# cmavro/GNN-RAG

Hardware: AMD Instinct MI355X
Metric: kg_edges_aggregated_per_sec (higher is better)
Workload: dtype f32

## Files before the change

### gnn-rag_amd/csrc/dense_internal.h

```cpp
#pragma once
#include "gnnrag_common.h"

namespace gnnrag {

int tables_vq_launch_z(const gnnrag_csr* csr, const void* planes, const float* ins, const float* W, float* P, int32_t D,
                       int32_t I, int32_t only_dir, float* zero, int64_t zero_n, hipStream_t stream);

int tables_vq_lite_launch_z(const gnnrag_csr* csr, const void* planes, const float* ins, const float* W, float* P, int32_t D,
                            int32_t I, int32_t only_dir, float* zero, int64_t zero_n, hipStream_t stream);

int update_b3_launch_z(const float* h, const float* nbr, const float* W, const float* b, const float* w_s,
                       const float* b_s, const float* mask, float* h_out, float* score, int64_t BN, int32_t D,
                       int32_t ldw, hipStream_t stream, bool score_zeroed);

int update_score_fused_rows(const float* h, const float* nbr, const uint8_t* add_flag, const float* W, const float* b,
                            const float* w_s, const float* b_s, const float* mask, float* h_out, float* score,
                            int64_t BN, int32_t D, int32_t I, int32_t math, hipStream_t stream, bool score_zeroed);
int update_b3_launch_f(const float* h, const float* nbr, const uint8_t* add_flag, const float* W, const float* b,
                       const float* w_s, const float* b_s, const float* mask, float* h_out, float* score, int64_t BN,
                       int32_t D, int32_t ldw, hipStream_t stream, bool score_zeroed);

bool update_rows_supported(const float* h, const float* nbr, const float* W, const float* h_out, int64_t BN, int32_t D,
                           int32_t I, int32_t math);
bool update_b3_shape_ok(int64_t BN, int32_t D, int32_t ldw);
int tables_small_launch(const gnnrag_csr* csr, const float* T_fwd, const float* T_inv, const float* ins, const float* W,
                        float* P, int32_t D, int32_t I, hipStream_t stream);

int frontier_build_z(const gnnrag_csr* csr, const float* dist, void* fws, size_t fws_bytes, float* zero_a,
                     int64_t zero_na, float* zero_b, int64_t zero_nb, hipStream_t stream);
const uint8_t* frontier_row_flags(const gnnrag_csr* csr, const void* fws);

int update_score_fused_z(const float* h, const float* nbr, const float* W, const float* b, const float* w_s,
                         const float* b_s, const float* mask, float* h_out, float* score, int64_t BN, int32_t D,
                         int32_t I, int32_t math, hipStream_t stream, bool score_zeroed);

bool rel_transform_accepts(const float* relfeat_fwd, const float* relfeat_inv, int64_t R1, int32_t D, int32_t L,
                           const gnnrag_layer_params* layers, int32_t pos_rows, const float* T_out, const void* planes_out);

}
```

### gnn-rag_amd/csrc/gemm_f32.hip

```cpp
#include "gnnrag_common.h"
#include "dense_internal.h"

#define GNNRAG_GEMM_MT1_NW 8
#ifndef GNNRAG_UPDATE_B3
#define GNNRAG_UPDATE_B3 1
#endif
#ifndef GNNRAG_TABLES_WRES
#define GNNRAG_TABLES_WRES 1
#endif
#ifndef GNNRAG_GEMM_WRES
#define GNNRAG_GEMM_WRES 1
#endif
#ifndef GNNRAG_UPDATE_SKINNY
#define GNNRAG_UPDATE_SKINNY 1
#endif

namespace gnnrag {


constexpr int kBK = 32;
constexpr int kSkinnyMaxM = 16384;

enum { EPI_LINEAR = 0, EPI_UPDATE = 1 };

// ... 705 lines not shown
  for (int nt = 0; nt < NT; ++nt) wrow[nt] = g.W + (size_t)min(nt * 16 + fr, Nout - 1) * g.ldw + g.wc0;
  for (int k0 = 0; k0 < K; k0 += 32) {
    f32x4 a[2], b[2][NT];
#pragma unroll
    for (int c = 0; c < 2; ++c) {
      const int k = k0 + c * 16 + fg * 4;
      const bool ok = k < K;
      a[c] = ok ? *reinterpret_cast<const f32x4*>(arow + k) : zero4;
#pragma unroll
      for (int nt = 0; nt < NT; ++nt) b[c][nt] = ok ? *reinterpret_cast<const f32x4*>(wrow[nt] + k) : zero4;
    }
#pragma unroll
    for (int c = 0; c < 2; ++c)
#pragma unroll
      for (int nt = 0; nt < NT; ++nt)
#pragma unroll
        for (int e = 0; e < 4; ++e) acc[nt] = __builtin_amdgcn_mfma_f32_16x16x4f32(a[c][e], b[c][nt][e], acc[nt], 0, 0, 0);
  }
  const int rbase = m0 + 4 * fg;
  unsigned fl = 0x01010101u;
  if (g.add_flag) fl = *reinterpret_cast<const unsigned*>(g.add_flag + rbase);
  float part[4] = {0.f, 0.f, 0.f, 0.f};
#pragma unroll
  for (int nt = 0; nt < NT; ++nt) {
    const int col = nt * 16 + fr;
    const bool cok = col < Nout;
    const float bia = (cok && g.bias) ? g.bias[col] : 0.f;
    const float wsc = cok ? g.w_s[col] : 0.f;
#pragma unroll
    for (int q = 0; q < 4; ++q) {
      const int row = rbase + q;
      float v = 0.f;
      if (cok && row < g.M) {
        float ad = 0.f;
        if (g.add && ((fl >> (8 * q)) & 0xffu)) ad = g.add[(size_t)row * Nout + col];
        v = fmaxf((acc[nt][q] + bia) + ad, 0.f);
        g.C[(size_t)row * Nout + col] = v;
      }
      part[q] += v * wsc;
    }
  }
  const float tot = row16_sum4(part, lane);
  const int srow = rbase + row16_sum4_index(fr);
  if (fr < 4 && srow < g.M) g.score[srow] = (tot + g.b_s[0]) + (1.0f - g.mask[srow]) * kVeryNeg;
}

static bool update_skinny_ok(const GemmArgs& g) {
  return g.M < 4096 && !g.A1 && g.K == g.K0 && g.K % 4 == 0 && g.Nout <= 208 && g.ldw % 4 == 0 && g.wc0 % 4 == 0 &&
         aligned16(g.A0) && aligned16(g.W) && (!g.add || g.add_rows >= g.M) &&
         (!g.add_flag || ((uintptr_t)g.add_flag & 3) == 0);
}

static int launch_update_skinny(const GemmArgs& g, hipStream_t stream) {
  const int nt = (g.Nout + 15) / 16;
  const dim3 grid((unsigned)(((g.M + 15) / 16 + 3) / 4));
#define GNNRAG_USK(N) case N: hipLaunchKernelGGL((k_update_skinny<N>), grid, dim3(256), 0, stream, g); break;
  switch (nt) {
    GNNRAG_USK(1) GNNRAG_USK(2) GNNRAG_USK(3) GNNRAG_USK(4) GNNRAG_USK(5) GNNRAG_USK(6) GNNRAG_USK(7) GNNRAG_USK(8)
    GNNRAG_USK(9) GNNRAG_USK(10) GNNRAG_USK(11) GNNRAG_USK(12) GNNRAG_USK(13)
    default: return GNNRAG_E_UNSUPPORTED;
  }
#undef GNNRAG_USK
  GNNRAG_LAUNCH_CHECK();
  return 0;
}

static bool math_ok(int math) { return math == GNNRAG_MATH_FP32 || math == GNNRAG_MATH_BF16X3 || math == GNNRAG_MATH_MIXED; }

template <int EPI, int AMODE>
static int launch_gemm(GemmArgs g, hipStream_t stream, int math) {
  if (g.M <= 0) return 0;
  const bool v4 = (g.K % 4 == 0) && (g.K0 % 4 == 0) && (g.ldw % 4 == 0) && (g.wc0 % 4 == 0) &&
                  aligned16(g.A0) && aligned16(g.W) && (g.A1 == nullptr || aligned16(g.A1)) &&
                  (g.C_b == nullptr || aligned16(g.A0b)) &&
                  (AMODE != AMODE_GEN || g.gen_D % 4 == 0);
  if (EPI == EPI_LINEAR && AMODE == AMODE_PLAIN && g.M <= kSkinnyMaxM && g.n0 == 0) {
    const dim3 grid((g.M + 15) / 16, (g.Nout + 255) / 256, g.C_b ? 2 : 1);
    if (v4) hipLaunchKernelGGL((k_gemm_skinny<true>), grid, dim3(256), 0, stream, g);
    else hipLaunchKernelGGL((k_gemm_skinny<false>), grid, dim3(256), 0, stream, g);
    GNNRAG_LAUNCH_CHECK();
    return 1 << 30;
  }
  const int ny = AMODE == AMODE_GEN ? 2 : 1;
  const int tiles128 = ((g.M + 127) / 128) * ny;
  const bool small_tiles = tiles128 < 1024;
  const int slots8 = 512;
  const int t8 = tiles128;
  const bool nw8 = small_tiles && (t8 >= 3 * slots8 / 2 || (t8 % slots8 == 0) || (t8 % slots8) > slots8 / 2) &&
                   GNNRAG_GEMM_MT1_NW == 8;
  const int bm = small_tiles ? (nw8 ? 128 : 64) : 128;
  const dim3 grid((g.M + bm - 1) / bm, ny);
  const int ncol = g.Nout - g.n0;
  const bool b3 = math != GNNRAG_MATH_FP32;
  g.v4out = (g.Nout % 4 == 0) && (g.n0 % 4 == 0) && aligned16(g.C) && (g.add == nullptr || aligned16(g.add));
#define GNNRAG_GEMM_LAUNCH(NT, MT, V, MATH, NW) \
  hipLaunchKernelGGL((k_gemm_f32<NT, MT, V, EPI, AMODE, MATH, NW>), grid, dim3(64 * NW), 0, stream, g)
#define GNNRAG_GEMM_CASE(NT)                                                        \
  do {                                                                              \
    if (small_tiles && nw8) {                                                       \
      if (v4 && b3) GNNRAG_GEMM_LAUNCH(NT, 1, true, 1, 8);                          \
      else if (v4) GNNRAG_GEMM_LAUNCH(NT, 1, true, 0, 8);                           \
      else GNNRAG_GEMM_LAUNCH(NT, 1, false, 0, 8);                                  \
    } else if (small_tiles) {                                                       \
      if (v4 && b3) GNNRAG_GEMM_LAUNCH(NT, 1, true, 1, 4);                          \
      else if (v4) GNNRAG_GEMM_LAUNCH(NT, 1, true, 0, 4);                           \
      else GNNRAG_GEMM_LAUNCH(NT, 1, false, 0, 4);                                  \
    } else {                                                                        \
      if (v4 && b3) GNNRAG_GEMM_LAUNCH(NT, 2, true, 1, 4);                          \
      else if (v4) GNNRAG_GEMM_LAUNCH(NT, 2, true, 0, 4);                           \
      else GNNRAG_GEMM_LAUNCH(NT, 2, false, 0, 4);                                  \
    }                                                                               \
  } while (0)
  if (ncol <= 64) GNNRAG_GEMM_CASE(4);
  else if (ncol <= 128) GNNRAG_GEMM_CASE(8);
  else GNNRAG_GEMM_CASE(13);
#undef GNNRAG_GEMM_CASE
#undef GNNRAG_GEMM_LAUNCH
  GNNRAG_LAUNCH_CHECK();
  return 0;
}

}

using namespace gnnrag;


extern "C" int gnnrag_linear(const float* A, int64_t M, int32_t K, const float* W, const float* bias,
                             const float* add, int64_t add_rows, int relu, float* C, int32_t Nout,
                             int32_t math, gnnrag_stream_t stream) {
  if (!A || !W || !C || M < 0 || K <= 0 || Nout <= 0 || !math_ok(math)) return GNNRAG_E_BADARG;
  if (M >= ((int64_t)1 << 31)) return GNNRAG_E_UNSUPPORTED;
  GemmArgs g;
  memset(&g, 0, sizeof(g));
  g.A0 = A; g.W = W; g.bias = bias; g.add = add; g.C = C;
  g.M = (int32_t)M; g.K = K; g.K0 = K; g.Nout = Nout; g.ldw = K;
  g.add_rows = add ? (int32_t)(add_rows < M ? add_rows : M) : 0;
  g.relu = relu;
  for (int n0 = 0; n0 < Nout; n0 += 208) {
    g.n0 = n0;
    const int rc = launch_gemm<EPI_LINEAR, AMODE_PLAIN>(g, (hipStream_t)stream, math);
    if (rc == (1 << 30)) break;
    if (rc) return rc;
  }
  return 0;
}

static int update_common(GemmArgs g, int64_t BN, int32_t D, hipStream_t stream, int math, bool score_zeroed = false) {
  if (D <= 208) {
    g.n0 = 0;
    const bool al = aligned16(g.A0) && aligned16(g.W) && aligned16(g.C) && (!g.add || aligned16(g.add)) &&
                    g.ldw % 4 == 0 && g.wc0 % 4 == 0 && (!g.add || g.add_rows >= g.M);
    if (GNNRAG_UPDATE_B3 && math != GNNRAG_MATH_FP32 && al && g.add && !g.A1 && g.K == D &&
        (!g.add_flag || ((uintptr_t)g.add_flag & 3) == 0)) {
      const int rc = update_b3_launch_f(g.A0, g.add, g.add_flag, g.W, g.bias, g.w_s, g.b_s, g.mask, g.C, g.score, BN, D,
                                        g.ldw, stream, score_zeroed);
      if (rc != GNNRAG_E_UNSUPPORTED) return rc;
    }
    const int S = (GNNRAG_GEMM_WRES && math != GNNRAG_MATH_BF16X3 && al && g.M >= 4096 &&
                   (!g.add_flag || ((uintptr_t)g.add_flag & 3) == 0)) ? wres_stride(g) : 0;
    if (S) return launch_wres<EPI_UPDATE>(g, S, stream);
    if (GNNRAG_UPDATE_SKINNY && update_skinny_ok(g)) return launch_update_skinny(g, stream);
    if (g.add_flag) return GNNRAG_E_UNSUPPORTED;
    return launch_gemm<EPI_UPDATE, AMODE_PLAIN>(g, stream, math);
  }
  if (g.add_flag) return GNNRAG_E_UNSUPPORTED;
  g.relu = 1;
  for (int n0 = 0; n0 < D; n0 += 208) {
    g.n0 = n0;
    const int rc = launch_gemm<EPI_LINEAR, AMODE_PLAIN>(g, stream, math);
    if (rc == (1 << 30)) break;
    if (rc) return rc;
  }
  hipLaunchKernelGGL(k_score_rows, dim3((int)((BN + 3) / 4)), dim3(256), 0, stream, g.C, g.w_s, g.b_s, g.mask,
                     g.score, (int)BN, D);
  GNNRAG_LAUNCH_CHECK();
  return 0;
}

extern "C" int gnnrag_linear_pair(const float* A0, const float* A1, int64_t M, int32_t K, const float* W,
                                  const float* bias, const float* add0, const float* add1, int64_t add_rows,
                                  float* C0, float* C1, int32_t Nout, int32_t math, gnnrag_stream_t stream) {
  if (!A0 || !A1 || !W || !C0 || !C1 || M < 0 || K <= 0 || Nout <= 0 || !math_ok(math)) return GNNRAG_E_BADARG;
  if ((add0 == nullptr) != (add1 == nullptr)) return GNNRAG_E_BADARG;
  if (M > kSkinnyMaxM) {
    int rc = gnnrag_linear(A0, M, K, W, bias, add0, add_rows, 0, C0, Nout, math, stream);
    if (rc) return rc;
    return gnnrag_linear(A1, M, K, W, bias, add1, add_rows, 0, C1, Nout, math, stream);
  }
  GemmArgs g;
  memset(&g, 0, sizeof(g));
  g.A0 = A0; g.A0b = A1; g.W = W; g.bias = bias; g.add = add0; g.add_b = add1; g.C = C0; g.C_b = C1;
  g.M = (int32_t)M; g.K = K; g.K0 = K; g.Nout = Nout; g.ldw = K;
  g.add_rows = add0 ? (int32_t)(add_rows < M ? add_rows : M) : 0;
  const int rc = launch_gemm<EPI_LINEAR, AMODE_PLAIN>(g, (hipStream_t)stream, math);
  return rc == (1 << 30) ? 0 : rc;
}

extern "C" int gnnrag_update_score(const float* h, const float* agg, const float* W, const float* b,
                                   const float* w_s, const float* b_s, const float* mask, float* h_out,
                                   float* score, int64_t BN, int32_t D, int32_t I, int32_t math,
                                   gnnrag_stream_t stream) {
  if (!h || !agg || !W || !b || !w_s || !b_s || !mask || !h_out || !score || BN < 0 || D <= 0 || I <= 0 ||
      !math_ok(math))
    return GNNRAG_E_BADARG;
  if (BN >= ((int64_t)1 << 31)) return GNNRAG_E_UNSUPPORTED;
  GemmArgs g;
  memset(&g, 0, sizeof(g));
  g.A0 = h; g.A1 = agg; g.W = W; g.bias = b; g.C = h_out;
  g.w_s = w_s; g.b_s = b_s; g.mask = mask; g.score = score;
  g.M = (int32_t)BN; g.K = (2 * I + 1) * D; g.K0 = D; g.Nout = D; g.ldw = g.K;
  g.relu = 1;
  return update_common(g, BN, D, (hipStream_t)stream, math);
}

extern "C" int gnnrag_update_score_fused(const float* h, const float* nbr, const float* W, const float* b,
                                         const float* w_s, const float* b_s, const float* mask, float* h_out,
                                         float* score, int64_t BN, int32_t D, int32_t I, int32_t math,
                                         gnnrag_stream_t stream) {
  return gnnrag::update_score_fused_z(h, nbr, W, b, w_s, b_s, mask, h_out, score, BN, D, I, math, (hipStream_t)stream,
                                      false);
}

bool gnnrag::update_rows_supported(const float* h, const float* nbr, const float* W, const float* h_out, int64_t BN,
                                   int32_t D, int32_t I, int32_t math) {
  if (D > 208 || BN >= ((int64_t)1 << 31)) return false;
  const int ldw = (2 * I + 1) * D;
  const bool al = aligned16(h) && aligned16(W) && aligned16(h_out) && aligned16(nbr) && ldw % 4 == 0;
  if (!al) return false;
  if (GNNRAG_UPDATE_B3 && math != GNNRAG_MATH_FP32 && update_b3_shape_ok(BN, D, ldw)) return true;
  if (GNNRAG_UPDATE_SKINNY && BN < 4096 && D % 4 == 0) return true;
  if (!(GNNRAG_GEMM_WRES && math != GNNRAG_MATH_BF16X3 && BN >= 4096)) return false;
  GemmArgs g;
  memset(&g, 0, sizeof(g));
  g.M = (int32_t)BN; g.K = D; g.K0 = D; g.Nout = D; g.ldw = ldw;
  return wres_stride(g) != 0;
}

int gnnrag::update_score_fused_z(const float* h, const float* nbr, const float* W, const float* b, const float* w_s,
                                 const float* b_s, const float* mask, float* h_out, float* score, int64_t BN, int32_t D,
                                 int32_t I, int32_t math, hipStream_t stream, bool score_zeroed) {
  return update_score_fused_rows(h, nbr, nullptr, W, b, w_s, b_s, mask, h_out, score, BN, D, I, math, stream, score_zeroed);
}

int gnnrag::update_score_fused_rows(const float* h, const float* nbr, const uint8_t* add_flag, const float* W,
                                    const float* b, const float* w_s, const float* b_s, const float* mask, float* h_out,
                                    float* score, int64_t BN, int32_t D, int32_t I, int32_t math, hipStream_t stream,
                                    bool score_zeroed) {
  if (!h || !nbr || !W || !b || !w_s || !b_s || !mask || !h_out || !score || BN < 0 || D <= 0 || I <= 0 ||
      !math_ok(math))
    return GNNRAG_E_BADARG;
  if (BN >= ((int64_t)1 << 31)) return GNNRAG_E_UNSUPPORTED;
  GemmArgs g;
  memset(&g, 0, sizeof(g));
  g.A0 = h; g.W = W; g.bias = b; g.add = nbr; g.add_rows = (int32_t)BN; g.C = h_out;
  g.w_s = w_s; g.b_s = b_s; g.mask = mask; g.score = score;
  g.M = (int32_t)BN; g.K = D; g.K0 = D; g.Nout = D; g.ldw = (2 * I + 1) * D; g.wc0 = 0;
  g.relu = 1;
  g.add_flag = add_flag;
  return update_common(g, BN, D, stream, math, score_zeroed);
}

extern "C" int gnnrag_relation_tables(const gnnrag_csr* csr, const float* T_fwd, const float* T_inv,
                                      const float* ins, const float* W, float* P, int32_t D, int32_t I,
                                      int32_t math, gnnrag_stream_t stream) {
  if (!csr || !T_fwd || !T_inv || !ins || !W || !P || D <= 0 || I <= 0 || csr->rel_total < 0 || !math_ok(math))
    return GNNRAG_E_BADARG;
  if (csr->rel_total == 0) return 0;
  {
    const int rc = tables_small_launch(csr, T_fwd, T_inv, ins, W, P, D, I, (hipStream_t)stream);
    if (rc != GNNRAG_E_UNSUPPORTED) return rc;
  }
  if (math == GNNRAG_MATH_MIXED) math = GNNRAG_MATH_BF16X3;
  if (math == GNNRAG_MATH_BF16X3 && GNNRAG_TABLES_WRES) {
    const int rc = tables_b3_launch(csr, T_fwd, T_inv, ins, W, P, D, I, (hipStream_t)stream);
    if (rc != GNNRAG_E_UNSUPPORTED) return rc;
  }
  GemmArgs g;
  memset(&g, 0, sizeof(g));
  g.A0 = T_fwd;
  g.A0b = T_inv;
  g.A1 = ins;
  g.W = W;
  g.C = P;
  g.M = csr->rel_total; g.K = I * D; g.K0 = g.K; g.Nout = D; g.ldw = (2 * I + 1) * D;
  g.gen_rows = (const int2*)csr->rel_rows; g.gen_D = D; g.gen_I = I;
  for (int n0 = 0; n0 < D; n0 += 208) {
    g.n0 = n0;
    const int rc = launch_gemm<EPI_LINEAR, AMODE_GEN>(g, (hipStream_t)stream, math);
    if (rc) return rc;
  }
  return 0;
}
```

### gnn-rag_amd/csrc/tables_b3.hip

```cpp
#include "gnnrag_common.h"
#include "dense_internal.h"

namespace gnnrag {

#ifndef GNNRAG_TAB_TPW
#define GNNRAG_TAB_TPW 3
#endif
#ifndef GNNRAG_TAB_MINBLK
#define GNNRAG_TAB_MINBLK 2
#endif
constexpr int kTabTPW = GNNRAG_TAB_TPW;
constexpr int kTabNTH = 7;
constexpr int kTabNKB = 7;
constexpr int kTabSlots = 26;
constexpr int kTabQBytes = 160 * 1024 - 3 * kTabNTH * 16 * kTabSlots * 16 - 64;

struct TabArgs {
  const float* T[2];
  const float* ins;
  const float* W;
  float* P;
  const int2* rows;
  int32_t M, D, I, ldw;
  int32_t ct0;
// ... 698 lines not shown
          *reinterpret_cast<uint2*>(dst + PL) = sp.mid;
          *reinterpret_cast<uint2*>(dst + 2 * PL) = sp.lo;
        }
      }
    }
  }
  const long long U = ((long long)a.M + 15) >> 4;
  const int c0 = (int)(U * chunk / nchunks), c1 = (int)(U * (chunk + 1) / nchunks);
  const int nch = c1 - c0;
  int t = c0 + (int)((long long)nch * wave / 8);
  const int tend = c0 + (int)((long long)nch * (wave + 1) / 8);
  const int kmax = D - 8;
  const unsigned char* Ab = reinterpret_cast<const unsigned char*>(a.A);
  const unsigned char* addb = reinterpret_cast<const unsigned char*>(a.add);
  unsigned char* Cb = reinterpret_cast<unsigned char*>(a.C);
  const unsigned rowB = (unsigned)D * 4u;
  const unsigned k6B = (unsigned)min(32 * (NKB - 1) + 8 * fg, kmax) * 4u;
  auto a_rowoff = [&](int tile) -> unsigned { return (unsigned)min(tile * 16 + fr, a.M - 1) * rowB; };
  auto a_piece = [&](unsigned rowoff, int kb, int half) -> f32x4 {
    const unsigned off = kb < NKB - 1 ? rowoff + 32u * (unsigned)fg + (unsigned)(128 * kb + 16 * half)
                                      : rowoff + k6B + (unsigned)(16 * half);
    return *reinterpret_cast<const f32x4*>(Ab + off);
  };
  f32x4 ra[NKB][2];
  if (t < tend) {
    const unsigned ro = a_rowoff(t);
#pragma unroll
    for (int kb = 0; kb < NKB; ++kb) {
      ra[kb][0] = a_piece(ro, kb, 0);
      ra[kb][1] = a_piece(ro, kb, 1);
    }
  }
  const float bs = a.b_s[0];
  const unsigned cgB = (unsigned)(col0 + min(4 * fr, ncol - 4)) * 4u;
  unsigned ctB[CTN > 4 ? CTN - 4 : 1];
#pragma unroll
  for (int nt = 4; nt < CTN; ++nt) ctB[nt - 4] = (unsigned)(col0 + min(nt * 16 + fr, ncol - 1)) * 4u;
  unsigned fl_next = 0x01010101u;
  if (FL && t < tend) fl_next = *reinterpret_cast<const unsigned*>(a.add_flag + (size_t)t * 16 + 4 * fg);
  __syncthreads();

  for (; t < tend; ++t) {
    const int rbase = t * 16 + 4 * fg;
    const unsigned fl = fl_next;
    if (FL) fl_next = *reinterpret_cast<const unsigned*>(a.add_flag + (size_t)(t + 1 < tend ? t + 1 : t) * 16 + 4 * fg);
    f32x4 addg[4];
    float addt[CTN > 4 ? CTN - 4 : 1][4];
#pragma unroll
    for (int q = 0; q < 4; ++q) {
      int row = min(rbase + q, a.M - 1);
      if (FL && ((fl >> (8 * q)) & 0xffu) == 0u) row = a.M;
      const unsigned ro = (unsigned)row * rowB;
      addg[q] = *reinterpret_cast<const f32x4*>(addb + (ro + cgB));
#pragma unroll
      for (int nt = 4; nt < CTN; ++nt) addt[nt - 4][q] = *reinterpret_cast<const float*>(addb + (ro + ctB[nt - 4]));
    }
    float mrow = 0.f;
    {
      const int srow = min(rbase + (2 * (fr & 1) + ((fr >> 1) & 1)), a.M - 1);
      mrow = a.mask[srow];
    }
    __builtin_amdgcn_sched_barrier(0);
    f32x4 acc[CTN];
#pragma unroll
    for (int nt = 0; nt < CTN; ++nt) acc[nt] = zero4;
    const unsigned ro_next = a_rowoff(t + 1 < tend ? t + 1 : t);
    const unsigned char* wbp[3];
#pragma unroll
    for (int pl = 0; pl < 3; ++pl) {
      unsigned o = (unsigned)(fr * RB + fg * 16 + pl * PL);
      asm volatile("" : "+v"(o));
      wbp[pl] = lds + o;
    }
    constexpr int PA[6] = {1, 2, 0, 1, 0, 0};
    constexpr int PB[6] = {1, 0, 2, 0, 1, 0};
#pragma unroll
    for (int kb = 0; kb < NKB; ++kb) {
      typedef unsigned u32x4 __attribute__((ext_vector_type(4)));
      bf16x8 ap[3];
      const bool kok = kb < NKB - 1 || 32 * kb + 8 * fg <= kmax;
      const Split3 s0 = split3(kok ? ra[kb][0] : zero4);
      const Split3 s1 = split3(kok ? ra[kb][1] : zero4);
      ap[0] = __builtin_bit_cast(bf16x8, (u32x4){s0.hi.x, s0.hi.y, s1.hi.x, s1.hi.y});
      ap[1] = __builtin_bit_cast(bf16x8, (u32x4){s0.mid.x, s0.mid.y, s1.mid.x, s1.mid.y});
      ap[2] = __builtin_bit_cast(bf16x8, (u32x4){s0.lo.x, s0.lo.y, s1.lo.x, s1.lo.y});
      ra[kb][0] = a_piece(ro_next, kb, 0);
      ra[kb][1] = a_piece(ro_next, kb, 1);
#pragma unroll
      for (int nt = 0; nt < CTN; nt += 2) {
        bf16x8 b0[3], b1[3];
#pragma unroll
        for (int pl = 0; pl < 3; ++pl) {
          b0[pl] = __builtin_bit_cast(bf16x8, *reinterpret_cast<const f32x4*>(wbp[pl] + (nt * 16 * RB + kb * 64)));
          b1[pl] = b0[pl];
          if (nt + 1 < CTN)
            b1[pl] = __builtin_bit_cast(bf16x8, *reinterpret_cast<const f32x4*>(wbp[pl] + ((nt + 1) * 16 * RB + kb * 64)));
        }
#pragma unroll
        for (int p = 0; p < 6; ++p) {
          acc[nt] = __builtin_amdgcn_mfma_f32_16x16x32_bf16(ap[PA[p]], b0[PB[p]], acc[nt], 0, 0, 0);
          if (nt + 1 < CTN)
            acc[nt + 1] = __builtin_amdgcn_mfma_f32_16x16x32_bf16(ap[PA[p]], b1[PB[p]], acc[nt + 1], 0, 0, 0);
        }
      }
    }
    float part[4] = {0.f, 0.f, 0.f, 0.f};
    const f32x4 bias_g = *reinterpret_cast<const f32x4*>(Bl + min(4 * fr, kTabNTH * 16 - 4));
    const f32x4 ws_g = *reinterpret_cast<const f32x4*>(Sl + min(4 * fr, kTabNTH * 16 - 4));
#pragma unroll
    for (int q = 0; q < 4; ++q) {
      const int row = rbase + q;
      const unsigned ro = (unsigned)min(row, a.M - 1) * rowB;
      f32x4 v = {acc[0][q], acc[1][q], acc[2][q], acc[3][q]};
      v = __builtin_elementwise_max((v + bias_g) + addg[q], zero4);
      const int c = 4 * fr;
      if (c + 4 > ncol) {
        v = zero4;
      } else if (row < a.M) {
        *reinterpret_cast<f32x4*>(Cb + (ro + cgB)) = v;
      }
      part[q] += v[0] * ws_g[0] + v[1] * ws_g[1] + v[2] * ws_g[2] + v[3] * ws_g[3];
#pragma unroll
      for (int nt = 4; nt < CTN; ++nt) {
        const int cc = nt * 16 + fr;
        float x = fmaxf((acc[nt][q] + Bl[cc]) + addt[nt - 4][q], 0.f);
        if (cc >= ncol) x = 0.f;
        else if (row < a.M) *reinterpret_cast<float*>(Cb + (ro + ctB[nt - 4])) = x;
        part[q] += x * Sl[cc];
      }
    }
    {
      const float tot = row16_sum4_b3(part, lane);
      const int srow = rbase + (2 * (fr & 1) + ((fr >> 1) & 1));
      if (fr < 4 && srow < a.M) {
        const float share = first_part ? (tot + bs) + (1.0f - mrow) * kVeryNeg : tot;
        atomicAdd(a.score + srow, share);
      }
    }
  }
}

template <bool FL>
__global__ __launch_bounds__(512, 2) void k_update_b3(UpdB3Args a, int nchunks) {
  extern __shared__ __attribute__((aligned(16))) unsigned char lds[];
  const int blk = blockIdx.x;
  const int NT = (a.D + 15) >> 4;
  const int h = (blk >> 3) & 1;
  const int chunk = (blk >> 4) * 8 + (blk & 7);
  if (chunk >= nchunks) return;
  if (h == 0) update_b3_part<kTabNTH, FL>(a, lds, 0, true, chunk, nchunks);
  else if (NT - a.ct0 == 6) update_b3_part<6, FL>(a, lds, a.ct0 * 16, false, chunk, nchunks);
}

int update_b3_launch(const float* h, const float* nbr, const float* W, const float* b, const float* w_s, const float* b_s,
                     const float* mask, float* h_out, float* score, int64_t BN, int32_t D, int32_t ldw,
                     hipStream_t stream) {
  return update_b3_launch_z(h, nbr, W, b, w_s, b_s, mask, h_out, score, BN, D, ldw, stream, false);
}

int update_b3_launch_z(const float* h, const float* nbr, const float* W, const float* b, const float* w_s,
                       const float* b_s, const float* mask, float* h_out, float* score, int64_t BN, int32_t D,
                       int32_t ldw, hipStream_t stream, bool score_zeroed) {
  return update_b3_launch_f(h, nbr, nullptr, W, b, w_s, b_s, mask, h_out, score, BN, D, ldw, stream, score_zeroed);
}

bool update_b3_shape_ok(int64_t BN, int32_t D, int32_t ldw) {
  return !(D % 8 || (D + 31) / 32 != kTabNKB || (D + 15) / 16 != 13 || BN < 8192 || (BN + 1) * D * 4 >= ((int64_t)1 << 32) || ldw % 4);
}

int update_b3_launch_f(const float* h, const float* nbr, const uint8_t* add_flag, const float* W, const float* b,
                       const float* w_s, const float* b_s, const float* mask, float* h_out, float* score, int64_t BN,
                       int32_t D, int32_t ldw, hipStream_t stream, bool score_zeroed) {
  if (!update_b3_shape_ok(BN, D, ldw)) return GNNRAG_E_UNSUPPORTED;
  if ((((uintptr_t)h | (uintptr_t)nbr | (uintptr_t)W | (uintptr_t)h_out) & 15) != 0) return GNNRAG_E_UNSUPPORTED;
  UpdB3Args a;
  memset(&a, 0, sizeof(a));
  a.A = h; a.W = W; a.bias = b; a.add = nbr; a.w_s = w_s; a.b_s = b_s; a.mask = mask; a.C = h_out; a.score = score;
  a.M = (int32_t)BN; a.D = D; a.ldw = ldw; a.ct0 = kTabNTH;
  a.add_flag = add_flag;
  if (add_flag && ((uintptr_t)add_flag & 3)) return GNNRAG_E_UNSUPPORTED;
  int cus = 0;
  {
    const int rc = device_cu_count(&cus);
    if (rc) return rc;
  }
  const long long U = (BN + 15) / 16;
  int chunks = cus / 2;
  if (chunks < 1) chunks = 1;
  if ((long long)chunks * 8 > U) chunks = (int)((U + 7) / 8);
  if (!score_zeroed) GNNRAG_HIP(hipMemsetAsync(score, 0, (size_t)BN * sizeof(float), stream));
  static DeviceMask cap, cap_f;
  {
    const int rc = add_flag ? raise_lds_cap(k_update_b3<true>, cap_f) : raise_lds_cap(k_update_b3<false>, cap);
    if (rc) return rc;
  }
  const int nblk = ((chunks + 7) / 8) * 16;
  if (add_flag) hipLaunchKernelGGL(k_update_b3<true>, dim3(nblk), dim3(512), 160 * 1024, stream, a, chunks);
  else hipLaunchKernelGGL(k_update_b3<false>, dim3(nblk), dim3(512), 160 * 1024, stream, a, chunks);
  GNNRAG_LAUNCH_CHECK();
  return 0;
}

size_t tables_vq_planes_bytes(int64_t R1) { return (size_t)2 * 3 * R1 * kVqRowB; }

bool tables_vq_shape_ok(int32_t D, int32_t I) {
  return D % 8 == 0 && (D + 31) / 32 == kTabNKB && (D + 15) / 16 == 13 && I >= 1 &&
         (size_t)I * D * sizeof(float) <= (size_t)kTabQBytes;
}

int tables_vq_launch(const gnnrag_csr* csr, const void* planes, const float* ins, const float* W, float* P, int32_t D,
                     int32_t I, int32_t only_dir, hipStream_t stream) {
  return tables_vq_launch_z(csr, planes, ins, W, P, D, I, only_dir, nullptr, 0, stream);
}

int tables_vq_launch_z(const gnnrag_csr* csr, const void* planes, const float* ins, const float* W, float* P, int32_t D,
                       int32_t I, int32_t only_dir, float* zero, int64_t zero_n, hipStream_t stream) {
  if (!tables_vq_shape_ok(D, I) || csr->rel_total < 1024 || only_dir > 1) return GNNRAG_E_UNSUPPORTED;
  if ((((uintptr_t)planes | (uintptr_t)ins | (uintptr_t)W | (uintptr_t)P) & 15) != 0) return GNNRAG_E_UNSUPPORTED;
  VqArgs a;
  memset(&a, 0, sizeof(a));
  a.planes = (const unsigned char*)planes; a.ins = ins; a.W = W; a.P = P;
  a.rows = (const int2*)csr->rel_rows; a.rel_off = csr->rel_off;
  a.M = csr->rel_total; a.D = D; a.I = I; a.ldw = (2 * I + 1) * D; a.R1 = csr->R1;
  const int NT = (D + 15) / 16;
  a.ct0 = (NT + 1) / 2;
  int cus = 0;
  {
    const int rc = device_cu_count(&cus);
    if (rc) return rc;
  }
  const int ndir = only_dir < 0 ? 2 : 1;
  a.dir0 = only_dir < 0 ? 0 : only_dir;
  int nchunk = cus / (csr->B * 2 * ndir);
  const int tiles_max = (csr->rel_max + 15) / 16;
  if (nchunk > tiles_max / 8) nchunk = tiles_max / 8;
  if (nchunk < 1) nchunk = 1;
  a.nchunk = nchunk;
  a.zero = zero;
  a.zero_n = zero ? zero_n : 0;
  static DeviceMask cap;
  {
    const int rc = raise_lds_cap(k_tables_vq, cap);
    if (rc) return rc;
  }
  hipLaunchKernelGGL(k_tables_vq, dim3(csr->B * nchunk, ndir, 2), dim3(512), 160 * 1024, stream, a);
  GNNRAG_LAUNCH_CHECK();
  return 0;
}

int tables_vq_lite_launch_z(const gnnrag_csr* csr, const void* planes, const float* ins, const float* W, float* P, int32_t D,
                            int32_t I, int32_t only_dir, float* zero, int64_t zero_n, hipStream_t stream) {
  if (!tables_vq_shape_ok(D, I) || csr->rel_total < 1024 || only_dir > 1) return GNNRAG_E_UNSUPPORTED;
  if ((((uintptr_t)planes | (uintptr_t)ins | (uintptr_t)W | (uintptr_t)P) & 15) != 0) return GNNRAG_E_UNSUPPORTED;
  VqArgs a;
  memset(&a, 0, sizeof(a));
  a.planes = (const unsigned char*)planes; a.ins = ins; a.W = W; a.P = P;
  a.rows = (const int2*)csr->rel_rows; a.rel_off = csr->rel_off;
  a.M = csr->rel_total; a.D = D; a.I = I; a.ldw = (2 * I + 1) * D; a.R1 = csr->R1;
  a.ct0 = kVlCT;
  int cus = 0;
  {
    const int rc = device_cu_count(&cus);
    if (rc) return rc;
  }
  const int ndir = only_dir < 0 ? 2 : 1;
  a.dir0 = only_dir < 0 ? 0 : only_dir;
  int nchunk = cus / (csr->B * 5 * ndir);
  const int tiles_max = (csr->rel_max + 15) / 16;
  if (nchunk > tiles_max / 8) nchunk = tiles_max / 8;
  if (nchunk < 1) nchunk = 1;
  a.nchunk = nchunk;
  a.zero = zero;
  a.zero_n = zero ? zero_n : 0;
  static DeviceMask cap;
  {
    const int rc = raise_lds_cap(k_tables_vq_lite, cap);
    if (rc) return rc;
  }
  size_t lds = (size_t)3 * kVlCT * 16 * kTabSlots * 16 + 64 + (size_t)I * D * sizeof(float);
  if (const char* e = getenv("GNNRAG_VL_LDS_KB")) {
    const size_t want = (size_t)atoi(e) * 1024;
    if (want > lds && want <= 160 * 1024) lds = want;
  }
  hipLaunchKernelGGL(k_tables_vq_lite, dim3(csr->B * nchunk, ndir, 5), dim3(kVlThreads), lds, stream, a);
  GNNRAG_LAUNCH_CHECK();
  return 0;
}

int tables_b3_launch(const gnnrag_csr* csr, const float* T_fwd, const float* T_inv, const float* ins, const float* W,
                     float* P, int32_t D, int32_t I, hipStream_t stream) {
  if (D % 8 || (D + 31) / 32 != kTabNKB || (D + 15) / 16 != 13 || csr->rel_total < 1024) return GNNRAG_E_UNSUPPORTED;
  if ((((uintptr_t)T_fwd | (uintptr_t)T_inv | (uintptr_t)ins | (uintptr_t)W | (uintptr_t)P) & 15) != 0)
    return GNNRAG_E_UNSUPPORTED;
  TabArgs a;
  memset(&a, 0, sizeof(a));
  a.T[0] = T_fwd; a.T[1] = T_inv; a.ins = ins; a.W = W; a.P = P;
  a.rows = (const int2*)csr->rel_rows;
  a.M = csr->rel_total; a.D = D; a.I = I; a.ldw = (2 * I + 1) * D;
  const int NT = (D + 15) / 16;
  a.ct0 = NT <= kTabNTH ? NT : (NT + 1) / 2;
  const int parts = NT <= kTabNTH ? 1 : 2;
  int cus = 0;
  {
    const int rc = device_cu_count(&cus);
    if (rc) return rc;
  }
  const long long U = ((long long)a.M + 15) / 16;
  int chunks = cus / (2 * parts);
  if (chunks < 1) chunks = 1;
  if ((long long)chunks * 8 > U) chunks = (int)((U + 7) / 8);
  const int tiles_per_wave = (int)((((U + chunks - 1) / chunks) + 7) / 8);
  a.npass = (tiles_per_wave + kTabTPW - 1) / kTabTPW;
  const size_t lds = 160 * 1024;
  static DeviceMask cap;
  {
    const int rc = raise_lds_cap(k_tables_b3, cap);
    if (rc) return rc;
  }
  hipLaunchKernelGGL(k_tables_b3, dim3(chunks, 2, parts), dim3(512), lds, stream, a);
  GNNRAG_LAUNCH_CHECK();
  return 0;
}

}

extern "C" int gnnrag_relation_tables_planes(const gnnrag_csr* csr, const void* planes, const float* ins, const float* W,
                                             float* P, int32_t D, int32_t I, gnnrag_stream_t stream) {
  if (!csr || !planes || !ins || !W || !P || D <= 0 || I <= 0 || csr->rel_total < 0) return GNNRAG_E_BADARG;
  if (csr->rel_total == 0) return 0;
  return gnnrag::tables_vq_launch(csr, planes, ins, W, P, D, I, -1, (hipStream_t)stream);
}
```

### gnn-rag_amd/ops.py

```python
from __future__ import annotations

import ctypes as C
import os
from typing import Optional

import numpy as np
import torch

from . import _lib


MATH_FP32, MATH_BF16X3, MATH_MIXED = 0, 1, 2
MATH_NAMES = {MATH_FP32: "fp32 (v_mfma_f32_16x16x4_f32, bit-exact fmaf chains)",
              MATH_BF16X3: "bf16x3 (exact 3-way bf16 split, 6 plane products on v_mfma_f32_16x16x32_bf16, fp32 accumulate)",
              MATH_MIXED: "mixed (per kernel the faster fp32-class form: bf16x3 - exact 3-way bf16 split, 6 plane products, "
                          "fp32 accumulate - for the relation tables and the self-block update, exact fp32 MFMA for the "
                          "small products)"}
_default_math = {"fp32": MATH_FP32, "bf16x3": MATH_BF16X3, "mixed": MATH_MIXED}[os.environ.get("GNNRAG_MATH", "mixed")]


def set_dense_math(mode: int) -> int:
    global _default_math
    if mode not in (MATH_FP32, MATH_BF16X3, MATH_MIXED):
        raise ValueError("unknown math mode %r" % (mode,))
    old, _default_math = _default_math, int(mode)
    return old


def get_dense_math() -> int:
    return _default_math


def _math(math: Optional[int]) -> int:
    return _default_math if math is None else int(math)


def _stream() -> int:
    return torch.cuda.current_stream().cuda_stream


def _ptr(t: Optional[torch.Tensor]) -> Optional[int]:
    return None if t is None else t.data_ptr()


def _chk(t: torch.Tensor, name: str, dtype=torch.float32, shape=None) -> torch.Tensor:
    if not t.is_cuda:
        raise _lib.GnnragError("%s must live on the GPU (got %s); there is no CPU path" % (name, t.device))
    if t.dtype != dtype:
        raise TypeError("%s must be %s, got %s" % (name, dtype, t.dtype))
    if not t.is_contiguous():
        t = t.contiguous()
    if shape is not None and tuple(t.shape) != tuple(shape):
        raise ValueError("%s has shape %s, expected %s" % (name, tuple(t.shape), tuple(shape)))
    return t


_stage_buf = {"t": None}


def _pinned_stage(n: int) -> torch.Tensor:
    t = _stage_buf["t"]
    if t is None or t.numel() < n:
        t = torch.empty(max(n, 1 << 20, 0 if t is None else 2 * t.numel()), dtype=torch.int32, pin_memory=True)
        _stage_buf["t"] = t
    return t


def _on_plan_device(plan: "CsrPlan", t: torch.Tensor, name: str) -> None:
    if t.device != plan.device and not (t.is_cuda and plan.device.index is None):
        raise _lib.GnnragError("%s lives on %s but the structure was built on %s" % (name, t.device, plan.device))


class CsrPlan:

    def __init__(self, heads, rels, tails, B: int, N: int, R1: int, device, validate: bool = True,
                 hrt_device: Optional[torch.Tensor] = None, rel_counts=None):
        lib = _lib.load()
        if hrt_device is not None:
            if (hrt_device.dtype != torch.int32 or hrt_device.dim() != 2 or hrt_device.shape[0] != 3
                    or not hrt_device.is_cuda or not hrt_device.is_contiguous()):
                raise ValueError("hrt_device must be a contiguous [3, F] int32 CUDA tensor")
            heads = rels = tails = None
            F = int(hrt_device.shape[1])
        else:
            heads = np.asarray(heads)
            rels = np.asarray(rels)
            tails = np.asarray(tails)
            F = int(heads.shape[0])
        if hrt_device is None and (rels.shape[0] != F or tails.shape[0] != F):
            raise ValueError("heads/rels/tails differ in length")
        if B <= 0 or N <= 0 or R1 <= 0:
            raise ValueError("B, N, R1 must be positive")
        if B * N >= 2 ** 31 or F >= 2 ** 31:
            raise ValueError("batch too large for int32 indices")
        self.B, self.N, self.R1, self.F = int(B), int(N), int(R1), F
        self.device = torch.device(device)
        if self.device.type != "cuda":
            raise _lib.GnnragError("CsrPlan needs a GPU device, got %s" % self.device)
        if self.device.index is None:
            self.device = torch.device("cuda", torch.cuda.current_device())
        base = None if hrt_device is not None else heads.base
        if hrt_device is not None:
            if hrt_device.device != self.device and not (self.device.index is None):
                raise _lib.GnnragError("hrt_device lives on %s, the plan on %s" % (hrt_device.device, self.device))
            hrt = hrt_device if F else torch.zeros((3, 1), dtype=torch.int32, device=hrt_device.device)
        elif (F and isinstance(base, np.ndarray) and heads.dtype == np.int32 and base is rels.base
                and base is tails.base and base.dtype == np.int32 and base.shape == (3, F) and base.flags.c_contiguous
                and heads.ctypes.data == base[0].ctypes.data and rels.ctypes.data == base[1].ctypes.data
                and tails.ctypes.data == base[2].ctypes.data and heads.shape == rels.shape == tails.shape == (F,)
                and heads.strides == rels.strides == tails.strides == (4,)):
            hrt = base
        elif (F and heads.dtype == rels.dtype == tails.dtype == np.int64 and heads.flags.c_contiguous
              and rels.flags.c_contiguous and tails.flags.c_contiguous):
            stage = _pinned_stage(3 * F)
            rc = lib.gnnrag_narrow_tuple(heads.ctypes.data, rels.ctypes.data, tails.ctypes.data, F, stage.data_ptr(),
                                         min(8, os.cpu_count() or 1))
            if rc == _lib.E_TUPLE:
                raise ValueError("edge tuple out of range: ids must lie in [0, 2^31)")
            _lib.check(rc, "gnnrag_narrow_tuple")
            hrt = stage[: 3 * F].view(3, F)
        else:
            for name, a in (("heads", heads), ("rels", rels), ("tails", tails)):
                if F and a.dtype.itemsize > 4 and (int(a.max()) >= 2 ** 31 or int(a.min()) < 0):
                    raise ValueError("edge tuple out of range: %s holds ids outside [0, 2^31)" % name)
            hrt = np.empty((3, max(F, 1)), dtype=np.int32)
            hrt[0, :F], hrt[1, :F], hrt[2, :F] = heads, rels, tails
        with torch.cuda.device(self.device):
            if hrt_device is not None:
                self._hrt = hrt
            elif isinstance(hrt, np.ndarray):
                self._hrt = torch.from_numpy(hrt).to(self.device, non_blocking=False)
            else:
                self._hrt = hrt.to(self.device, non_blocking=True)
                torch.cuda.current_stream().synchronize()
            nbytes = lib.gnnrag_csr_bytes(F, B, N, R1, 0, 0)
            sbytes = lib.gnnrag_csr_scratch_bytes(F, B, N, R1)
            self._mem = torch.empty(max(nbytes, 256), dtype=torch.uint8, device=self.device)
            scratch = torch.empty(max(sbytes, 256), dtype=torch.uint8, device=self.device)
            self.c = _lib.CsrStruct()
            row = self._hrt
            rt, rm = (-1, -1) if rel_counts is None else (int(rel_counts[0]), int(rel_counts[1]))
            rc = lib.gnnrag_csr_build_counts(
                row[0].data_ptr(), row[1].data_ptr(), row[2].data_ptr(), None, None,
                F, B, N, R1, rt, rm, self._mem.data_ptr(), self._mem.numel(),
                scratch.data_ptr(), scratch.numel(), C.byref(self.c), _stream())
            if rel_counts is not None:
                scratch.record_stream(torch.cuda.current_stream())
            if rc == _lib.E_TUPLE:
                raise ValueError("edge tuple out of range: node ids must lie in [0, B*N), relation ids in [0, R1), "
                                 "and a fact may not connect two different questions")
            _lib.check(rc, "gnnrag_csr_build")
        self._w = {}
        self.rel_total, self.rel_max = int(self.c.rel_total), int(self.c.rel_max)

    def status(self) -> None:
        rc = _lib.load().gnnrag_csr_status(C.byref(self.c), _stream())
        if rc == _lib.E_TUPLE:
            raise ValueError("edge tuple out of range: node ids must lie in [0, B*N), relation ids in [0, R1), "
                             "and a fact may not connect two different questions")
        _lib.check(rc, "gnnrag_csr_status (relation counts passed to the build differ from the device's)")

    @classmethod
    def concat(cls, parts, N: int, R1: int, device) -> "CsrPlan":
        lib = _lib.load()
        B = len(parts)
        if B == 0:
            raise ValueError("a batch needs at least one question")
        self = cls.__new__(cls)
        self.B, self.N, self.R1 = B, int(N), int(R1)
        self.F = int(sum(p.F for p in parts))
# ... 802 lines not shown
```

Baseline: 2.891 billion.

## Use scaled fp16x2 split MFMA for self-block update in mixed mode

Adds a new update kernel that splits A and W into two fp16 planes, hi and lo, with power-of-two per-row and per-column scaling. It runs three plane products on 16x16x32 f16 MFMA in place of the bf16x3 scheme's six products on three planes. The new kernel is selected for the default mixed math mode and halves the LDS weight planes. The aim is to cut MFMA work and LDS footprint in the self-block update, at the cost of lower precision than the exact 3-way split.

```diff
diff --git a/gnn-rag_amd/csrc/dense_internal.h b/gnn-rag_amd/csrc/dense_internal.h
--- a/gnn-rag_amd/csrc/dense_internal.h
+++ b/gnn-rag_amd/csrc/dense_internal.h
@@ -20,6 +20,10 @@
                        const float* w_s, const float* b_s, const float* mask, float* h_out, float* score, int64_t BN,
                        int32_t D, int32_t ldw, hipStream_t stream, bool score_zeroed);
 
+int update_h2_launch_f(const float* h, const float* nbr, const uint8_t* add_flag, const float* W, const float* b,
+                       const float* w_s, const float* b_s, const float* mask, float* h_out, float* score, int64_t BN,
+                       int32_t D, int32_t ldw, hipStream_t stream, bool score_zeroed);
+
 bool update_rows_supported(const float* h, const float* nbr, const float* W, const float* h_out, int64_t BN, int32_t D,
                            int32_t I, int32_t math);
 bool update_b3_shape_ok(int64_t BN, int32_t D, int32_t ldw);
diff --git a/gnn-rag_amd/csrc/gemm_f32.hip b/gnn-rag_amd/csrc/gemm_f32.hip
--- a/gnn-rag_amd/csrc/gemm_f32.hip
+++ b/gnn-rag_amd/csrc/gemm_f32.hip
@@ -881,8 +881,8 @@
                     g.ldw % 4 == 0 && g.wc0 % 4 == 0 && (!g.add || g.add_rows >= g.M);
     if (GNNRAG_UPDATE_B3 && math != GNNRAG_MATH_FP32 && al && g.add && !g.A1 && g.K == D &&
         (!g.add_flag || ((uintptr_t)g.add_flag & 3) == 0)) {
-      const int rc = update_b3_launch_f(g.A0, g.add, g.add_flag, g.W, g.bias, g.w_s, g.b_s, g.mask, g.C, g.score, BN, D,
-                                        g.ldw, stream, score_zeroed);
+      const int rc = (math == GNNRAG_MATH_MIXED ? update_h2_launch_f : update_b3_launch_f)(
+          g.A0, g.add, g.add_flag, g.W, g.bias, g.w_s, g.b_s, g.mask, g.C, g.score, BN, D, g.ldw, stream, score_zeroed);
       if (rc != GNNRAG_E_UNSUPPORTED) return rc;
     }
     const int S = (GNNRAG_GEMM_WRES && math != GNNRAG_MATH_BF16X3 && al && g.M >= 4096 &&
diff --git a/gnn-rag_amd/csrc/tables_b3.hip b/gnn-rag_amd/csrc/tables_b3.hip
--- a/gnn-rag_amd/csrc/tables_b3.hip
+++ b/gnn-rag_amd/csrc/tables_b3.hip
@@ -874,6 +874,256 @@
   else if (NT - a.ct0 == 6) update_b3_part<6, FL>(a, lds, a.ct0 * 16, false, chunk, nchunks);
 }
 
+typedef _Float16 f16x2_t __attribute__((ext_vector_type(2)));
+typedef _Float16 f16x8 __attribute__((ext_vector_type(8)));
+struct Split2 { uint2 hi, lo; };
+__device__ __forceinline__ unsigned pack_f16_rn(float a, float b) {
+  return __builtin_bit_cast(unsigned, __builtin_convertvector((f32x2){a, b}, f16x2_t));
+}
+__device__ __forceinline__ Split2 split2_f16(f32x4 x) {
+  const unsigned h01 = pack_f16_rn(x[0], x[1]), h23 = pack_f16_rn(x[2], x[3]);
+  const f16x2_t a = __builtin_bit_cast(f16x2_t, h01), b = __builtin_bit_cast(f16x2_t, h23);
+  Split2 s;
+  s.hi = make_uint2(h01, h23);
+  s.lo = make_uint2(pack_f16_rn(x[0] - (float)a[0], x[1] - (float)a[1]), pack_f16_rn(x[2] - (float)b[0], x[3] - (float)b[1]));
+  return s;
+}
+__device__ __forceinline__ int h2_exp(float m) {
+  return m > 0.f ? min(127, max(-126, 15 - __builtin_amdgcn_frexp_expf(m))) : 0;
+}
+__device__ __forceinline__ float pow2f(int s) { return __uint_as_float((unsigned)(s + 127) << 23); }
+
+template <int CTN, bool FL>
+__device__ __forceinline__ void update_h2_part(const UpdB3Args& a, unsigned char* lds, int col0, bool first_part,
+                                               int chunk, int nchunks) {
+  constexpr int RB = kTabSlots * 16;
+  constexpr int PL = kTabNTH * 16 * RB;
+  constexpr int NKB = kTabNKB;
+  const int tid = threadIdx.x, lane = tid & 63, wave = tid >> 6;
+  const int fr = lane & 15, fg = lane >> 4;
+  const int D = a.D;
+  const int ncol = min(CTN * 16, D - col0);
+  const int KC = D >> 2;
+  const f32x4 zero4 = {0.f, 0.f, 0.f, 0.f};
+  float* Bl = reinterpret_cast<float*>(lds + 2 * PL + 64);
+  float* Sl = Bl + kTabNTH * 16;
+  unsigned* Mx = reinterpret_cast<unsigned*>(Sl + kTabNTH * 16);
+
+  if (tid < 16) reinterpret_cast<unsigned*>(lds + 2 * PL)[tid] = 0u;
+  for (int j = tid; j < kTabNTH * 16; j += 512) {
+    Bl[j] = (j < ncol && a.bias) ? a.bias[col0 + j] : 0.f;
+    Sl[j] = j < ncol ? a.w_s[col0 + j] : 0.f;
+    Mx[j] = 0u;
+  }
+  __syncthreads();
+  for (int idx = tid; idx < ncol * KC; idx += 512) {
+    const int j = idx / KC, kc = idx - j * KC;
+    const f32x4 v = *reinterpret_cast<const f32x4*>(a.W + (size_t)(col0 + j) * a.ldw + 4 * kc);
+    const float m = fmaxf(fmaxf(fabsf(v[0]), fabsf(v[1])), fmaxf(fabsf(v[2]), fabsf(v[3])));
+    atomicMax(Mx + j, __float_as_uint(m));
+  }
+  __syncthreads();
+  {
+    const int total = tab_stage_rows(CTN) * kTabSlots * 2;
+    constexpr int UN = 6;
+    for (int base = 0; base < total; base += 512 * UN) {
+      f32x4 v[UN];
+      int off[UN];
+#pragma unroll
+      for (int u = 0; u < UN; ++u) {
+        const int idx = base + u * 512 + tid;
+        const int j = idx / (kTabSlots * 2), kc = idx - j * (kTabSlots * 2);
+        v[u] = zero4;
+        off[u] = idx < total ? tab_lds_row(j) * RB + kc * 8 : -1;
+        if (idx < total && j < ncol && kc < KC)
+          v[u] = *reinterpret_cast<const f32x4*>(a.W + (size_t)(col0 + j) * a.ldw + 4 * kc) *
+                 pow2f(h2_exp(__uint_as_float(Mx[j])));
+      }
+#pragma unroll
+      for (int u = 0; u < UN; ++u) {
+        if (off[u] >= 0) {
+          const Split2 sp = split2_f16(v[u]);
+          unsigned char* dst = lds + off[u];
+          *reinterpret_cast<uint2*>(dst) = sp.hi;
+          *reinterpret_cast<uint2*>(dst + PL) = sp.lo;
+        }
+      }
+    }
+  }
+  const long long U = ((long long)a.M + 15) >> 4;
+  const int c0 = (int)(U * chunk / nchunks), c1 = (int)(U * (chunk + 1) / nchunks);
+  const int nch = c1 - c0;
+  int t = c0 + (int)((long long)nch * wave / 8);
+  const int tend = c0 + (int)((long long)nch * (wave + 1) / 8);
+  const int kmax = D - 8;
+  const unsigned char* Ab = reinterpret_cast<const unsigned char*>(a.A);
+  const unsigned char* addb = reinterpret_cast<const unsigned char*>(a.add);
+  unsigned char* Cb = reinterpret_cast<unsigned char*>(a.C);
+  const unsigned rowB = (unsigned)D * 4u;
+  const unsigned k6B = (unsigned)min(32 * (NKB - 1) + 8 * fg, kmax) * 4u;
+  auto a_rowoff = [&](int tile) -> unsigned { return (unsigned)min(tile * 16 + fr, a.M - 1) * rowB; };
+  auto a_piece = [&](unsigned rowoff, int kb, int half) -> f32x4 {
+    const unsigned off = kb < NKB - 1 ? rowoff + 32u * (unsigned)fg + (unsigned)(128 * kb + 16 * half)
+                                      : rowoff + k6B + (unsigned)(16 * half);
+    return *reinterpret_cast<const f32x4*>(Ab + off);
+  };
+  f32x4 ra[NKB][2];
+  if (t < tend) {
+    const unsigned ro = a_rowoff(t);
+#pragma unroll
+    for (int kb = 0; kb < NKB; ++kb) {
+      ra[kb][0] = a_piece(ro, kb, 0);
+      ra[kb][1] = a_piece(ro, kb, 1);
+    }
+  }
+  const float bs = a.b_s[0];
+  const unsigned cgB = (unsigned)(col0 + min(4 * fr, ncol - 4)) * 4u;
+  unsigned ctB[CTN > 4 ? CTN - 4 : 1];
+#pragma unroll
+  for (int nt = 4; nt < CTN; ++nt) ctB[nt - 4] = (unsigned)(col0 + min(nt * 16 + fr, ncol - 1)) * 4u;
+  int nsb[CTN];
+#pragma unroll
+  for (int nt = 0; nt < CTN; ++nt) nsb[nt] = -h2_exp(__uint_as_float(Mx[nt < 4 ? 4 * fr + nt : nt * 16 + fr]));
+  unsigned fl_next = 0x01010101u;
+  if (FL && t < tend) fl_next = *reinterpret_cast<const unsigned*>(a.add_flag + (size_t)t * 16 + 4 * fg);
+  __syncthreads();
+
+  for (; t < tend; ++t) {
+    const int rbase = t * 16 + 4 * fg;
+    const unsigned fl = fl_next;
+    if (FL) fl_next = *reinterpret_cast<const unsigned*>(a.add_flag + (size_t)(t + 1 < tend ? t + 1 : t) * 16 + 4 * fg);
+    f32x4 addg[4];
+    float addt[CTN > 4 ? CTN - 4 : 1][4];
+#pragma unroll
+    for (int q = 0; q < 4; ++q) {
+      int row = min(rbase + q, a.M - 1);
+      if (FL && ((fl >> (8 * q)) & 0xffu) == 0u) row = a.M;
+      const unsigned ro = (unsigned)row * rowB;
+      addg[q] = *reinterpret_cast<const f32x4*>(addb + (ro + cgB));
+#pragma unroll
+      for (int nt = 4; nt < CTN; ++nt) addt[nt - 4][q] = *reinterpret_cast<const float*>(addb + (ro + ctB[nt - 4]));
+    }
+    float mrow = 0.f;
+    {
+      const int srow = min(rbase + (2 * (fr & 1) + ((fr >> 1) & 1)), a.M - 1);
+      mrow = a.mask[srow];
+    }
+    __builtin_amdgcn_sched_barrier(0);
+    int sa;
+    {
+      float m = 0.f;
+#pragma unroll
+      for (int kb = 0; kb < NKB; ++kb)
+#pragma unroll
+        for (int hf = 0; hf < 2; ++hf)
+#pragma unroll
+          for (int e = 0; e < 4; ++e) m = fmaxf(m, fabsf(ra[kb][hf][e]));
+      const auto s32 = __builtin_amdgcn_permlane32_swap(__float_as_uint(m), __float_as_uint(m), false, false);
+      m = fmaxf(__uint_as_float(s32[0]), __uint_as_float(s32[1]));
+      const auto s16 = __builtin_amdgcn_permlane16_swap(__float_as_uint(m), __float_as_uint(m), false, false);
+      m = fmaxf(__uint_as_float(s16[0]), __uint_as_float(s16[1]));
+      sa = h2_exp(m);
+    }
+    const float sca = pow2f(sa);
+    int nsa[4];
+#pragma unroll
+    for (int q = 0; q < 4; ++q) nsa[q] = -__shfl(sa, 4 * fg + q);
+    f32x4 acc[CTN];
+#pragma unroll
+    for (int nt = 0; nt < CTN; ++nt) acc[nt] = zero4;
+    const unsigned ro_next = a_rowoff(t + 1 < tend ? t + 1 : t);
+    const unsigned char* wbp[2];
+#pragma unroll
+    for (int pl = 0; pl < 2; ++pl) {
+      unsigned o = (unsigned)(fr * RB + fg * 16 + pl * PL);
+      asm volatile("" : "+v"(o));
+      wbp[pl] = lds + o;
+    }
+    constexpr int PA[3] = {1, 0, 0};
+    constexpr int PB[3] = {0, 1, 0};
+#pragma unroll
+    for (int kb = 0; kb < NKB; ++kb) {
+      typedef unsigned u32x4 __attribute__((ext_vector_type(4)));
+      f16x8 ap[2];
+      const bool kok = kb < NKB - 1 || 32 * kb + 8 * fg <= kmax;
+      const Split2 s0 = split2_f16(kok ? ra[kb][0] * sca : zero4);
+      const Split2 s1 = split2_f16(kok ? ra[kb][1] * sca : zero4);
+      ap[0] = __builtin_bit_cast(f16x8, (u32x4){s0.hi.x, s0.hi.y, s1.hi.x, s1.hi.y});
+      ap[1] = __builtin_bit_cast(f16x8, (u32x4){s0.lo.x, s0.lo.y, s1.lo.x, s1.lo.y});
+      ra[kb][0] = a_piece(ro_next, kb, 0);
+      ra[kb][1] = a_piece(ro_next, kb, 1);
+#pragma unroll
+      for (int nt = 0; nt < CTN; nt += 2) {
+        f16x8 b0[2], b1[2];
+#pragma unroll
+        for (int pl = 0; pl < 2; ++pl) {
+          b0[pl] = __builtin_bit_cast(f16x8, *reinterpret_cast<const f32x4*>(wbp[pl] + (nt * 16 * RB + kb * 64)));
+          b1[pl] = b0[pl];
+          if (nt + 1 < CTN)
+            b1[pl] = __builtin_bit_cast(f16x8, *reinterpret_cast<const f32x4*>(wbp[pl] + ((nt + 1) * 16 * RB + kb * 64)));
+        }
+#pragma unroll
+        for (int p = 0; p < 3; ++p) {
+          acc[nt] = __builtin_amdgcn_mfma_f32_16x16x32_f16(ap[PA[p]], b0[PB[p]], acc[nt], 0, 0, 0);
+          if (nt + 1 < CTN)
+            acc[nt + 1] = __builtin_amdgcn_mfma_f32_16x16x32_f16(ap[PA[p]], b1[PB[p]], acc[nt + 1], 0, 0, 0);
+        }
+      }
+    }
+#pragma unroll
+    for (int nt = 0; nt < CTN; ++nt)
+#pragma unroll
+      for (int q = 0; q < 4; ++q) acc[nt][q] = __builtin_amdgcn_ldexpf(acc[nt][q], nsa[q] + nsb[nt]);
+    float part[4] = {0.f, 0.f, 0.f, 0.f};
+    const f32x4 bias_g = *reinterpret_cast<const f32x4*>(Bl + min(4 * fr, kTabNTH * 16 - 4));
+    const f32x4 ws_g = *reinterpret_cast<const f32x4*>(Sl + min(4 * fr, kTabNTH * 16 - 4));
+#pragma unroll
+    for (int q = 0; q < 4; ++q) {
+      const int row = rbase + q;
+      const unsigned ro = (unsigned)min(row, a.M - 1) * rowB;
+      f32x4 v = {acc[0][q], acc[1][q], acc[2][q], acc[3][q]};
+      v = __builtin_elementwise_max((v + bias_g) + addg[q], zero4);
+      const int c = 4 * fr;
+      if (c + 4 > ncol) {
+        v = zero4;
+      } else if (row < a.M) {
+        *reinterpret_cast<f32x4*>(Cb + (ro + cgB)) = v;
+      }
+      part[q] += v[0] * ws_g[0] + v[1] * ws_g[1] + v[2] * ws_g[2] + v[3] * ws_g[3];
+#pragma unroll
+      for (int nt = 4; nt < CTN; ++nt) {
+        const int cc = nt * 16 + fr;
+        float x = fmaxf((acc[nt][q] + Bl[cc]) + addt[nt - 4][q], 0.f);
+        if (cc >= ncol) x = 0.f;
+        else if (row < a.M) *reinterpret_cast<float*>(Cb + (ro + ctB[nt - 4])) = x;
+        part[q] += x * Sl[cc];
+      }
+    }
+    {
+      const float tot = row16_sum4_b3(part, lane);
+      const int srow = rbase + (2 * (fr & 1) + ((fr >> 1) & 1));
+      if (fr < 4 && srow < a.M) {
+        const float share = first_part ? (tot + bs) + (1.0f - mrow) * kVeryNeg : tot;
+        atomicAdd(a.score + srow, share);
+      }
+    }
+  }
+}
+
+constexpr size_t kUpdH2Lds = 2 * (size_t)kTabNTH * 16 * kTabSlots * 16 + 64 + 3 * kTabNTH * 16 * sizeof(float);
+
+template <bool FL>
+__global__ __launch_bounds__(512, 2) void k_update_h2(UpdB3Args a, int nchunks) {
+  extern __shared__ __attribute__((aligned(16))) unsigned char lds[];
+  const int blk = blockIdx.x;
+  const int NT = (a.D + 15) >> 4;
+  const int h = (blk >> 3) & 1;
+  const int chunk = (blk >> 4) * 8 + (blk & 7);
+  if (chunk >= nchunks) return;
+  if (h == 0) update_h2_part<kTabNTH, FL>(a, lds, 0, true, chunk, nchunks);
+  else if (NT - a.ct0 == 6) update_h2_part<6, FL>(a, lds, a.ct0 * 16, false, chunk, nchunks);
+}
+
 int update_b3_launch(const float* h, const float* nbr, const float* W, const float* b, const float* w_s, const float* b_s,
                      const float* mask, float* h_out, float* score, int64_t BN, int32_t D, int32_t ldw,
                      hipStream_t stream) {
@@ -890,9 +1140,9 @@
   return !(D % 8 || (D + 31) / 32 != kTabNKB || (D + 15) / 16 != 13 || BN < 8192 || (BN + 1) * D * 4 >= ((int64_t)1 << 32) || ldw % 4);
 }
 
-int update_b3_launch_f(const float* h, const float* nbr, const uint8_t* add_flag, const float* W, const float* b,
-                       const float* w_s, const float* b_s, const float* mask, float* h_out, float* score, int64_t BN,
-                       int32_t D, int32_t ldw, hipStream_t stream, bool score_zeroed) {
+static int update_wres_launch(const float* h, const float* nbr, const uint8_t* add_flag, const float* W, const float* b,
+                              const float* w_s, const float* b_s, const float* mask, float* h_out, float* score,
+                              int64_t BN, int32_t D, int32_t ldw, hipStream_t stream, bool score_zeroed, bool h2) {
   if (!update_b3_shape_ok(BN, D, ldw)) return GNNRAG_E_UNSUPPORTED;
   if ((((uintptr_t)h | (uintptr_t)nbr | (uintptr_t)W | (uintptr_t)h_out) & 15) != 0) return GNNRAG_E_UNSUPPORTED;
   UpdB3Args a;
@@ -911,16 +1161,34 @@
   if (chunks < 1) chunks = 1;
   if ((long long)chunks * 8 > U) chunks = (int)((U + 7) / 8);
   if (!score_zeroed) GNNRAG_HIP(hipMemsetAsync(score, 0, (size_t)BN * sizeof(float), stream));
-  static DeviceMask cap, cap_f;
+  static DeviceMask cap, cap_f, cap_h, cap_hf;
   {
-    const int rc = add_flag ? raise_lds_cap(k_update_b3<true>, cap_f) : raise_lds_cap(k_update_b3<false>, cap);
+    const int rc = h2 ? (add_flag ? raise_lds_cap(k_update_h2<true>, cap_hf) : raise_lds_cap(k_update_h2<false>, cap_h))
+                      : (add_flag ? raise_lds_cap(k_update_b3<true>, cap_f) : raise_lds_cap(k_update_b3<false>, cap));
     if (rc) return rc;
   }
   const int nblk = ((chunks + 7) / 8) * 16;
-  if (add_flag) hipLaunchKernelGGL(k_update_b3<true>, dim3(nblk), dim3(512), 160 * 1024, stream, a, chunks);
-  else hipLaunchKernelGGL(k_update_b3<false>, dim3(nblk), dim3(512), 160 * 1024, stream, a, chunks);
+  if (h2) {
+    if (add_flag) hipLaunchKernelGGL(k_update_h2<true>, dim3(nblk), dim3(512), kUpdH2Lds, stream, a, chunks);
+    else hipLaunchKernelGGL(k_update_h2<false>, dim3(nblk), dim3(512), kUpdH2Lds, stream, a, chunks);
+  } else {
+    if (add_flag) hipLaunchKernelGGL(k_update_b3<true>, dim3(nblk), dim3(512), 160 * 1024, stream, a, chunks);
+    else hipLaunchKernelGGL(k_update_b3<false>, dim3(nblk), dim3(512), 160 * 1024, stream, a, chunks);
+  }
   GNNRAG_LAUNCH_CHECK();
   return 0;
+}
+
+int update_b3_launch_f(const float* h, const float* nbr, const uint8_t* add_flag, const float* W, const float* b,
+                       const float* w_s, const float* b_s, const float* mask, float* h_out, float* score, int64_t BN,
+                       int32_t D, int32_t ldw, hipStream_t stream, bool score_zeroed) {
+  return update_wres_launch(h, nbr, add_flag, W, b, w_s, b_s, mask, h_out, score, BN, D, ldw, stream, score_zeroed, false);
+}
+
+int update_h2_launch_f(const float* h, const float* nbr, const uint8_t* add_flag, const float* W, const float* b,
+                       const float* w_s, const float* b_s, const float* mask, float* h_out, float* score, int64_t BN,
+                       int32_t D, int32_t ldw, hipStream_t stream, bool score_zeroed) {
+  return update_wres_launch(h, nbr, add_flag, W, b, w_s, b_s, mask, h_out, score, BN, D, ldw, stream, score_zeroed, true);
 }
 
 size_t tables_vq_planes_bytes(int64_t R1) { return (size_t)2 * 3 * R1 * kVqRowB; }
diff --git a/gnn-rag_amd/ops.py b/gnn-rag_amd/ops.py
--- a/gnn-rag_amd/ops.py
+++ b/gnn-rag_amd/ops.py
@@ -13,9 +13,9 @@
 MATH_FP32, MATH_BF16X3, MATH_MIXED = 0, 1, 2
 MATH_NAMES = {MATH_FP32: "fp32 (v_mfma_f32_16x16x4_f32, bit-exact fmaf chains)",
               MATH_BF16X3: "bf16x3 (exact 3-way bf16 split, 6 plane products on v_mfma_f32_16x16x32_bf16, fp32 accumulate)",
-              MATH_MIXED: "mixed (per kernel the faster fp32-class form: bf16x3 - exact 3-way bf16 split, 6 plane products, "
-                          "fp32 accumulate - for the relation tables and the self-block update, exact fp32 MFMA for the "
-                          "small products)"}
+              MATH_MIXED: "mixed (per kernel the fastest fp32-class form: scaled fp16x2 - power-of-two row / column "
+                          "exponents, 2 fp16 planes, 3 plane products, fp32 accumulate - for the self-block update, "
+                          "bf16x3 for the relation tables, exact fp32 MFMA for the small products)"}
 _default_math = {"fp32": MATH_FP32, "bf16x3": MATH_BF16X3, "mixed": MATH_MIXED}[os.environ.get("GNNRAG_MATH", "mixed")]
 
 
```

Result: no change. 2.882 billion, median of 3 (-0.3%).
